# facebookresearch/param

Hardware: AMD Instinct MI355X
Metric: EmbeddingBag lookups/s + achieved HBM GB/s; all-to-all bus-BW at 1/2/4/8 GPU (higher is better)
Workload: dtype f32

## Files before the change

### param_amd/csrc/capi.hip

```cpp
#include <atomic>
#include <cstdio>
#include <cstdlib>
#include <string>

#include "common.h"

namespace {

thread_local std::string g_last_error;

constexpr int kDefaultUnroll = 2;
std::atomic<int> g_unroll{0};
std::atomic<int> g_bags_per_block{0};
std::atomic<int> g_xcd_affine{-1};
std::atomic<int> g_nt_loads{-1};
std::atomic<int> g_stage_out{-1};
std::atomic<int> g_flat_target{-1};
std::atomic<int> g_flat_grid{-1};
constexpr int kDefaultRowPolicy = 3;

int fail(int code, const std::string& msg) {
    g_last_error = msg;
    return code;
}

int hip_fail(hipError_t rc, const char* what) {
    return fail(PM_ERR_HIP, std::string(what) + ": " + hipGetErrorString(rc));
}

struct FwdEnv {
    int stage;
    int flat;
    int flat_maxl;
    int flat_target;
    int flat_bags;
    int tile_major;
    int flat_compact;
};
const FwdEnv& fwd_env() {
    static const FwdEnv e = [] {
        auto num = [](const char* name, int dflt) { const char* v = getenv(name); return v ? atoi(v) : dflt; };
        FwdEnv r;
        const char* st = getenv("PARAM_AMD_FWD_STAGE");
        r.stage = (st && st[0] == '0') ? 0 : 1;
        r.flat = num("PARAM_AMD_FWD_FLAT", 1);
        r.flat_maxl = num("PARAM_AMD_FLAT_MAXL", 0);
        r.flat_target = num("PARAM_AMD_FLAT_TARGET", 256);
        r.flat_bags = num("PARAM_AMD_FLAT_BAGS", 256);
        r.tile_major = num("PARAM_AMD_FWD_TILE_MAJOR", -1);
        r.flat_compact = num("PARAM_AMD_FLAT_COMPACT", 1);
        return r;
    }();
    return e;
}

int flat_target_knob(const FwdEnv& env) { const int k = g_flat_target.load(); return k > 0 ? k : env.flat_target; }

bool dtype_is_weight(int d) { return d == PM_F32 || d == PM_BF16 || d == PM_F16; }

int make_params(const pm_embbag_batch* op, int elem_dtype, pm::KParams& p, bool forward = false) {
    if (!op) return fail(PM_ERR_INVALID, "op is NULL");
    if (op->num_tables < 1) return fail(PM_ERR_INVALID, "num_tables must be >= 1");
    if (!dtype_is_weight(elem_dtype)) return fail(PM_ERR_INVALID, "weight/dst dtype must be PM_F32, PM_BF16 or PM_F16");
    if (op->index_dtype != PM_I64 && op->index_dtype != PM_I32)
        return fail(PM_ERR_INVALID, "index_dtype must be PM_I64 or PM_I32");
    if (op->batch < 0 || op->num_indices < 0) return fail(PM_ERR_INVALID, "negative batch / num_indices");
    if (op->bag_begin < 0 || op->bag_count < 0 || op->bag_begin + op->bag_count > op->batch)
        return fail(PM_ERR_INVALID, "bag_begin/bag_count outside [0, batch]");
    if (!op->tables || !op->rows || !op->dims || !op->out_offsets)
        return fail(PM_ERR_INVALID, "tables/rows/dims/out_offsets must be device pointers");
    if (op->bag_count > 0 && !op->offsets) return fail(PM_ERR_INVALID, "offsets is NULL");
    if (op->num_indices > 0 && !op->indices) return fail(PM_ERR_INVALID, "indices is NULL");
    const int vec = (elem_dtype == PM_F32) ? 4 : 8;
    if (op->max_dim < 1 || op->max_dim % vec != 0)
        return fail(PM_ERR_UNSUPPORTED, "every dims[t] (and max_dim) must be a multiple of " +
                                            std::to_string(vec) + " for this element type");
    if (op->out_stride % 4 != 0) return fail(PM_ERR_UNSUPPORTED, "out_stride must be a multiple of 4 elements");
    if (op->min_dim < 0 || op->min_dim > op->max_dim || (op->min_dim > 0 && op->min_dim % vec != 0))
        return fail(PM_ERR_INVALID, "min_dim must be 0 (not given) or a multiple of the vector width in [1, max_dim]");
    if (op->fixed_pooling < 0 ||
        (op->fixed_pooling > 0 && op->fixed_pooling * op->batch * static_cast<int64_t>(op->num_tables) != op->num_indices))
        return fail(PM_ERR_INVALID, "fixed_pooling must be 0 or num_indices / (num_tables * batch)");

    const int G = pm::group_lanes(op->max_dim, vec);
    const int NG = pm::kBlock / G;
    int bpb = g_bags_per_block.load();
    if (bpb <= 0) {
        bpb = 4 * NG;
        {
            const int64_t tb = static_cast<int64_t>(op->num_tables) * op->batch;
            if (tb > 0 && op->num_indices < 12 * tb) bpb = NG;
        }
        const int64_t want_blocks = 256 * 8;
        while (bpb > NG && static_cast<int64_t>(op->num_tables) * ((op->bag_count + bpb - 1) / bpb) < want_blocks) bpb /= 2;
    }
    if (bpb < NG) bpb = NG;
    if (bpb > 1024) bpb = 1024;

    const int64_t tiles = (op->bag_count + bpb - 1) / bpb;
    if (tiles * op->num_tables > 0x7fffffffLL) return fail(PM_ERR_UNSUPPORTED, "grid too large");

    const int64_t total_bags = static_cast<int64_t>(op->num_tables) * op->batch;
    const int64_t avg_l = total_bags > 0 ? (op->num_indices + total_bags - 1) / total_bags : 0;
    int64_t cap = 2 * bpb * avg_l;
    cap = (cap + 255) / 256 * 256;
    if (cap < (op->per_sample_weights ? 2048 : 4096)) cap = op->per_sample_weights ? 2048 : 4096;
    if (cap > 4096) cap = 4096;

    p.tables = op->tables;
    p.rows = op->rows;
    p.dims = op->dims;
    p.out_offsets = op->out_offsets;
    p.indices = op->indices;
    p.offsets = op->offsets;
    p.psw = op->per_sample_weights;
    p.io = nullptr;
    p.out_stride = op->out_stride;
    p.B = op->batch;
    p.N = op->num_indices;
    p.bag_begin = op->bag_begin;
    p.bag_count = op->bag_count;
    p.T = op->num_tables;
    p.tiles_per_table = static_cast<int32_t>(tiles);
    p.bags_per_block = bpb;
    p.idx_cap = static_cast<int32_t>(cap);
    p.idx64 = op->index_dtype == PM_I64 ? 1 : 0;
    const int xa = g_xcd_affine.load();
    {
        const int64_t tb = static_cast<int64_t>(op->num_tables) * op->batch;
        const bool even_req = tb > 0 && op->num_indices % tb == 0;
        p.xcd_affine = xa == 0 ? 0 : (op->num_tables % pm::kXcds == 0 ? 1 : ((op->num_tables > 1 && even_req) ? 3 : 0));
        if (xa != 0 && op->table_group > 1 && op->num_tables > 1 && even_req) p.xcd_affine = 3;
    }
    const int nt = g_nt_loads.load();
    p.nt_loads = nt > 0 ? nt : 0;
    p.ordered = (total_bags > 0 && op->num_indices % total_bags != 0 && bpb > NG) ? 1 : 0;
    p.alpha = 1.0f;
    if (op->grad_block_shift < 0 || op->grad_block_shift > 31 || op->grad_block_extra < 0 || op->table_group < 0)
        return fail(PM_ERR_INVALID, "grad_block_shift must be in [0, 31], grad_block_extra and table_group >= 0");
    if (op->grad_block_shift == 0 && op->grad_block_extra != 0)
        return fail(PM_ERR_INVALID, "grad_block_extra needs grad_block_shift >= 1 (a block of one bag is the un-blocked layout)");
    if (op->grad_block_shift > 0 && (op->batch & ((static_cast<int64_t>(1) << op->grad_block_shift) - 1)) != 0)
        return fail(PM_ERR_INVALID, "batch must be a multiple of 2^grad_block_shift bags");
    p.gblk_shift = op->grad_block_shift > 0 ? op->grad_block_shift : 31;
    p.gblk_extra = op->grad_block_shift > 0 ? op->grad_block_extra : 0;
    p.out_bits = 0;
    p.stage_out = 0;
    p.stage_bags = 0;
    p.flat_bags = 0;
    p.flat_target = 0;
    p.flat_compact = 0;
    if (forward) {
        const FwdEnv& env = fwd_env();
        int want = g_stage_out.load();
        if (want < 0) want = env.stage;
        const bool even = total_bags > 0 && op->num_indices % total_bags == 0;
        if (want && even && !p.ordered && g_bags_per_block.load() <= 0) {
            while (bpb > NG && static_cast<int64_t>(bpb) * op->max_dim * 4 > 16384) bpb /= 2;
            if (static_cast<int64_t>(bpb) * op->max_dim * 4 <= 16384) {
                const int64_t tiles2 = (op->bag_count + bpb - 1) / bpb;
                if (tiles2 * op->num_tables <= 0x7fffffffLL) {
                    p.bags_per_block = bpb;
                    p.tiles_per_table = static_cast<int32_t>(tiles2);
                    p.stage_out = op->max_dim;
                    int64_t need = (2 * static_cast<int64_t>(bpb) * avg_l + 255) / 256 * 256;
                    if (need < 512) need = 512;
                    if (need < p.idx_cap) p.idx_cap = static_cast<int32_t>(need);
                }
            }
        } else if (want && even && !p.ordered && static_cast<int64_t>(bpb) * op->max_dim * 4 <= 16384) {
            p.stage_out = op->max_dim;
            int64_t need = (2 * static_cast<int64_t>(bpb) * avg_l + 255) / 256 * 256;
            if (need < 512) need = 512;
            if (need < p.idx_cap) p.idx_cap = static_cast<int32_t>(need);
        } else if (want && !even && !p.ordered && g_bags_per_block.load() <= 0 &&
                   static_cast<int64_t>(bpb) * op->max_dim * 4 <= 4096) {
            p.stage_out = op->max_dim;
        }
        p.stage_bags = p.bags_per_block;
        const int flat_env = env.flat;
        const bool flat_on = flat_env != 0;
        const int flat_maxl = env.flat_maxl;
        if (flat_on && even && avg_l <= (flat_maxl > 0 ? flat_maxl : flat_env == 2 ? 4 : 2) && !p.ordered && g_bags_per_block.load() <= 0 &&
            p.stage_out > 0) {
            const int64_t tiles_ng = (op->bag_count + NG - 1) / NG;
            if (tiles_ng * op->num_tables <= 0x7fffffffLL) {
                const int tgt2 = flat_target_knob(env);
                p.flat_bags = env.flat_bags < 32 ? 32 : (env.flat_bags > 1024 ? 1024 : env.flat_bags / NG * NG);
                p.flat_target = tgt2;
                p.tiles_per_table = static_cast<int32_t>(tiles_ng);
                p.stage_bags = NG;
                p.bags_per_block = p.flat_bags;
                if (p.idx_cap < 1024) p.idx_cap = 1024;
            }
        }
        if (flat_on && !even && !p.ordered && g_bags_per_block.load() <= 0 && bpb == NG && p.stage_out > 0) {
            const int cap_env = env.flat_bags;
            const int tgt_env = flat_target_knob(env);
            p.flat_bags = cap_env < NG ? NG : (cap_env > 1024 ? 1024 : cap_env / NG * NG);
            p.flat_target = tgt_env < 1 ? 1 : tgt_env;
            p.bags_per_block = p.flat_bags;
        }
        if (flat_on && op->min_dim > 0 && op->min_dim < op->max_dim && !p.ordered && g_bags_per_block.load() <= 0) {
            int need = (op->min_dim + vec - 1) / vec, g_min = 4;
            while (g_min < need) g_min <<= 1;
            if (g_min < G) {
                const int ng_max = pm::kBlock / g_min;
                const int64_t tiles_ng = (op->bag_count + NG - 1) / NG;
                if (tiles_ng * op->num_tables <= 0x7fffffffLL) {
                    if (p.flat_bags < ng_max) p.flat_bags = ng_max;
                    if (p.flat_bags < 256) p.flat_bags = 256;
                    if (p.flat_bags < 32) p.flat_bags = 32;
                    if (p.flat_target <= 0) p.flat_target = flat_target_knob(env) < 1 ? 1 : flat_target_knob(env);
                    p.tiles_per_table = static_cast<int32_t>(tiles_ng);
                    p.bags_per_block = p.flat_bags;
                    p.stage_out = op->max_dim;
                    p.stage_bags = NG;
                    int64_t cap2 = 2 * static_cast<int64_t>(ng_max) * avg_l;
                    if (cap2 < 2 * static_cast<int64_t>(p.flat_target)) cap2 = 2 * static_cast<int64_t>(p.flat_target);
                    cap2 = (cap2 + 255) / 256 * 256;
                    p.idx_cap = static_cast<int32_t>(cap2 < 1024 ? 1024 : (cap2 > 4096 ? 4096 : cap2));
                    if (p.xcd_affine == 3) p.xcd_affine = 0;
                }
            }
        }
        {
            int fg = g_flat_grid.load();
            if (fg < 0) fg = env.flat_compact;
            if (p.flat_bags > 0 && op->num_tables <= 1024 && fg > 0) {
                const int64_t n_slice = op->batch > 0 ? (op->num_indices * op->bag_count + op->batch - 1) / op->batch : 0;
                const int64_t by_lookups = (n_slice + p.flat_target - 1) / p.flat_target;
                const int64_t by_bags = static_cast<int64_t>(op->num_tables) * ((op->bag_count + p.flat_bags - 1) / p.flat_bags);
                int64_t est = (by_lookups > by_bags ? by_lookups : by_bags) * 5 / 4 + op->num_tables;
                if (est < 1024) est = 1024;
                if (est > (1 << 20)) est = 1 << 20;
                p.flat_compact = fg > 1 ? fg : static_cast<int32_t>(est);
            }
        }
        const int tm_env = env.tile_major;
        const bool uneven = total_bags > 0 && op->num_indices % total_bags != 0;
        if (p.xcd_affine != 1 && op->num_tables > 1 && tm_env > 0 && uneven) p.xcd_affine = 2;
    }
    return PM_OK;
}

int small_request_unroll(const pm_embbag_batch* op, const pm::KParams& p) {
    if (p.flat_bags > 0 || p.ordered) return kDefaultUnroll;
    const int64_t wgs = static_cast<int64_t>(p.T) * p.tiles_per_table;
    const int64_t bags = static_cast<int64_t>(op->num_tables) * op->batch;
    const int64_t avg_l = bags > 0 ? op->num_indices / bags : 0;
    if (wgs > 384) return kDefaultUnroll;
    return avg_l >= 8 ? 8 : (avg_l >= 4 ? 4 : kDefaultUnroll);
}

}

extern "C" {

int pm_abi_version(void) { return PM_ABI_VERSION; }

const char* pm_build_info(void) {
    return "libparam_amd gfx950 (CDNA4, wave64) hip " __VERSION__;
}

const char* pm_last_error(void) { return g_last_error.c_str(); }

int pm_set_tuning(int32_t unroll, int32_t bags_per_block, int32_t xcd_affine, int32_t nt_loads) {
    if (unroll != 0 && unroll != 1 && unroll != 2 && unroll != 3 && unroll != 4 && unroll != 6 && unroll != 8)
        return fail(PM_ERR_INVALID, "unroll must be 0, 1, 2, 3, 4, 6 or 8");
    if (bags_per_block < 0) return fail(PM_ERR_INVALID, "bags_per_block must be >= 0");
    g_unroll.store(unroll);
    g_bags_per_block.store(bags_per_block);
    g_xcd_affine.store(xcd_affine);
    g_nt_loads.store(nt_loads);
    return PM_OK;
}

int pm_set_forward_tuning(int32_t stage_out, int32_t flat_grid, int32_t flat_target) {
    if (stage_out < -1 || stage_out > 1) return fail(PM_ERR_INVALID, "stage_out must be -1, 0 or 1");
    if (flat_grid < -1 || flat_grid > (1 << 20)) return fail(PM_ERR_INVALID, "flat_grid must be -1 (default), 0, 1 or a workgroup count up to 2^20");
    if (flat_target < -1 || flat_target == 0 || flat_target > 4096) return fail(PM_ERR_INVALID, "flat_target must be -1 (default) or 1 .. 4096");
    g_stage_out.store(stage_out);
    g_flat_grid.store(flat_grid);
    g_flat_target.store(flat_target);
    return PM_OK;
}

int pm_set_backward_tuning(int32_t sort_impl, int32_t order, int32_t xcd_affine, int32_t max_phases) {
    if (sort_impl < -1 || sort_impl > 2 || order < -1 || order > 1 || xcd_affine < -1 || xcd_affine > 1)
        return fail(PM_ERR_INVALID, "sort_impl must be -1 .. 2, order / xcd_affine -1, 0 or 1");
#ifndef PM_ALTERNATES
    if (sort_impl > 0)
        return fail(PM_ERR_UNSUPPORTED, "sort_impl 1 (rocPRIM) and 2 (round 2's LSD sort) exist in the alternates build only "
                                        "(libparam_amd_alt.so: make -C param_amd/csrc alt)");
#endif
    if (max_phases != -1 && max_phases != 1 && max_phases != 2) return fail(PM_ERR_INVALID, "max_phases must be -1, 1 or 2");
    pm::set_backward_tuning(sort_impl, order, xcd_affine, max_phases);
    return PM_OK;
}

int pm_set_sort_tuning(int32_t mode) {
    if (mode < -1 || mode > 3) return fail(PM_ERR_INVALID, "mode must be -1, 0, 1, 2 or 3");
    pm::set_sort_tuning(mode);
    return PM_OK;
}

int pm_set_hybrid_tuning(int32_t enable, int64_t lookback_spin_cap) {
    if (enable < -1 || enable > 2) return fail(PM_ERR_INVALID, "enable must be -1 .. 2");
    if (lookback_spin_cap < 0 || lookback_spin_cap > 0xffffffffLL) return fail(PM_ERR_INVALID, "lookback_spin_cap must be in [0, 2^32)");
    pm::set_hybrid_tuning(enable, static_cast<uint32_t>(lookback_spin_cap));
    return PM_OK;
}

int pm_set_hybrid_rest(int32_t mode) {
    if (mode < -1 || mode > 1) return fail(PM_ERR_INVALID, "mode must be -1 (default), 0 or 1");
    pm::set_hybrid_rest(mode);
    return PM_OK;
}

int pm_set_hybrid_min_tiles(int32_t tiles) {
    if (tiles < -1) return fail(PM_ERR_INVALID, "tiles must be -1 (default) or >= 0");
    pm::set_hybrid_min_tiles(tiles);
    return PM_OK;
}

int pm_embbag_sort_status(const pm_embbag_batch* op, int64_t max_rows, const void* workspace, pm_sort_status* out, pm_stream_t stream) {
    pm::KParams p;
    int rc = make_params(op, op ? op->weight_dtype : -1, p);
    if (rc != PM_OK) return rc;
    if (max_rows < 1 || max_rows > (1LL << 31)) return fail(PM_ERR_INVALID, "max_rows must be in [1, 2^31]");
    if (!workspace || !out) return fail(PM_ERR_INVALID, "NULL argument");
    uint32_t v[6] = {0, 0, 0, 0, 0, 0};
    const hipError_t h = pm::sort_status(p, max_rows, op->max_dim, workspace, static_cast<hipStream_t>(stream), v);
    if (h == hipErrorInvalidValue) return fail(PM_ERR_INVALID, "no sort has been recorded for this workspace");
    if (h != hipSuccess) return hip_fail(h, "pm_embbag_sort_status");
    out->lookback_fallbacks = v[0];
    out->pairs_sorted = v[1];
    out->hybrid_tables = v[2];
    out->hybrid_launched = v[3];
    out->lds_pairs = v[4];
    out->lds_tables = v[5];
    return PM_OK;
}

#ifdef PM_ALTERNATES
int64_t pm_radix_sort_scratch_bytes(int64_t n_max) {
    if (n_max < 0 || n_max > 0xffffffffLL) return fail(PM_ERR_INVALID, "n_max must be in [0, 2^32)");
    return static_cast<int64_t>(pm::rs_scratch_bytes(static_cast<size_t>(n_max)));
}

int pm_radix_sort_pairs(void* keys_a, void* keys_b, uint32_t* vals_a, uint32_t* vals_b, int64_t n_max,
                        const uint32_t* d_count, int32_t key_bytes, int32_t begin_bit, int32_t end_bit, int64_t segment_len,
                        void* scratch, int64_t scratch_bytes, int32_t* result_in_b, pm_stream_t stream) {
    if (n_max < 0 || n_max > 0xffffffffLL) return fail(PM_ERR_INVALID, "n_max must be in [0, 2^32)");
    if (key_bytes != 4 && key_bytes != 8) return fail(PM_ERR_INVALID, "key_bytes must be 4 or 8");
    if (begin_bit < 0 || end_bit < begin_bit || end_bit > key_bytes * 8) return fail(PM_ERR_INVALID, "bad bit range");
    if (!result_in_b) return fail(PM_ERR_INVALID, "result_in_b is NULL");
    if (segment_len < 0 || (segment_len > 0 && (segment_len % 4096 != 0 || n_max % segment_len != 0 || d_count)))
        return fail(PM_ERR_INVALID, "segment_len must be 0 or a multiple of 4096 dividing n_max (and d_count NULL)");
    *result_in_b = pm::rs_num_passes(begin_bit, end_bit) % 2;
    if (n_max == 0) return PM_OK;
    if (!keys_a || !keys_b || !vals_a || !vals_b) return fail(PM_ERR_INVALID, "key / value buffers are NULL");
    if (!scratch || scratch_bytes < static_cast<int64_t>(pm::rs_scratch_bytes(static_cast<size_t>(n_max))))
        return fail(PM_ERR_INVALID, "scratch too small: need " + std::to_string(pm::rs_scratch_bytes(static_cast<size_t>(n_max))) + " bytes");
    hipError_t h = key_bytes == 4
        ? pm::rs_sort_pairs<uint32_t>(static_cast<uint32_t*>(keys_a), static_cast<uint32_t*>(keys_b), vals_a, vals_b,
                                      static_cast<size_t>(n_max), d_count, begin_bit, end_bit, scratch, static_cast<hipStream_t>(stream),
                                      static_cast<size_t>(segment_len))
        : pm::rs_sort_pairs<uint64_t>(static_cast<uint64_t*>(keys_a), static_cast<uint64_t*>(keys_b), vals_a, vals_b,
                                      static_cast<size_t>(n_max), d_count, begin_bit, end_bit, scratch, static_cast<hipStream_t>(stream),
                                      static_cast<size_t>(segment_len));
    if (h != hipSuccess) return hip_fail(h, "pm_radix_sort_pairs");
    return PM_OK;
}
#endif

static int rowquant_args_ok(int64_t n_rows, int32_t dim, int32_t bitwidth) {
    if (n_rows < 0) return fail(PM_ERR_INVALID, "n_rows is negative");
    if (bitwidth != 16 && bitwidth != 8 && bitwidth != 4 && bitwidth != 2) return fail(PM_ERR_INVALID, "bitwidth must be 16, 8, 4 or 2");
    if (dim < 8 || dim % 8 != 0 || dim > 512) return fail(PM_ERR_UNSUPPORTED, "dim must be a multiple of 8 in [8, 512]");
    return PM_OK;
}

static uintptr_t rowquant_align(int32_t bitwidth) { return bitwidth == 16 ? 16 : static_cast<uintptr_t>(bitwidth); }

int64_t pm_rows_quantized_bytes(int64_t n_rows, int32_t dim, int32_t bitwidth) {
    const int rc = rowquant_args_ok(n_rows, dim, bitwidth);
    if (rc != PM_OK) return rc;
    return n_rows * pm::rows_quantized_row_bytes(dim, bitwidth);
}

int pm_rows_quantize(const float* src, int64_t n_rows, int32_t dim, int32_t bitwidth, void* dst, pm_stream_t stream) {
    const int rc = rowquant_args_ok(n_rows, dim, bitwidth);
    if (rc != PM_OK) return rc;
// ... 462 lines not shown
```

### param_amd/csrc/common.h

```cpp
#pragma once

#include <hip/hip_runtime.h>
#include <stdint.h>

#include <string>

#include "param_amd.h"

namespace pm {

constexpr int kBlock = 256;
constexpr int kWave = 64;
constexpr int kXcds = 8;

typedef uint32_t u32x4 __attribute__((ext_vector_type(4)));
typedef float f32x4 __attribute__((ext_vector_type(4)));

#define PM_GLOBAL __attribute__((address_space(1)))
template <typename T>
__device__ __forceinline__ const PM_GLOBAL T* as_global(const void* p) { return (const PM_GLOBAL T*)(p); }
template <typename T>
__device__ __forceinline__ PM_GLOBAL T* as_global(void* p) { return (PM_GLOBAL T*)(p); }

struct KParams {
    const void* const* tables;
    const int64_t* rows;
    const int32_t* dims;
    const int64_t* out_offsets;
    const void* indices;
    const void* offsets;
    const float* psw;
    float* io;
    int64_t out_stride;
    int64_t B;
    int64_t N;
    int64_t bag_begin;
    int64_t bag_count;
    int32_t T;
    int32_t tiles_per_table;
    int32_t bags_per_block;
    int32_t idx_cap;
    int32_t idx64;
    int32_t xcd_affine;
    int32_t nt_loads;
    int32_t ordered;
    int32_t stage_out;
    int32_t stage_bags;
    int32_t out_bits;
    int32_t flat_bags;
    int32_t flat_target;
    int32_t flat_compact;
    int32_t gblk_shift;
    int64_t gblk_extra;
    float alpha;
};

__device__ __forceinline__ int64_t grad_bag_offset(int64_t bag, int64_t out_stride, int shift, int64_t extra) {
    int64_t o = bag * out_stride;
    if (__builtin_expect(extra != 0, 0)) o += (bag >> shift) * extra;
    return o;
}

__device__ __forceinline__ int64_t load_index(const void* p, int64_t i, int idx64) {
    return idx64 ? as_global<int64_t>(p)[i] : static_cast<int64_t>(as_global<int32_t>(p)[i]);
}

__device__ __forceinline__ int64_t bag_start_or_end(const KParams& p, int64_t g) {
    const int64_t TB = static_cast<int64_t>(p.T) * p.B;
    return (g < TB) ? load_index(p.offsets, g, p.idx64) : p.N;
}

__device__ __forceinline__ int xcd_contiguous_tile(int bid, int total) {
    const int q = total / kXcds, r = total % kXcds, x = bid % kXcds;
    return x * q + (x < r ? x : r) + bid / kXcds;
}

__device__ __forceinline__ void block_to_tile(const KParams& p, int& t, int& tile, int bid = blockIdx.x) {
    if (p.xcd_affine == 3) {
        const int g = xcd_contiguous_tile(bid, p.T * p.tiles_per_table);
        t = g / p.tiles_per_table;
        tile = g % p.tiles_per_table;
    } else if (p.xcd_affine == 2) {
        t = bid % p.T;
        tile = bid / p.T;
    } else if (p.xcd_affine) {
        const int xcd = bid % kXcds;
        const int slot = bid / kXcds;
        t = xcd + kXcds * (slot / p.tiles_per_table);
        tile = slot % p.tiles_per_table;
    } else {
        t = bid / p.tiles_per_table;
        tile = bid % p.tiles_per_table;
    }
}

template <bool WEIGHTED>
__device__ __forceinline__ bool stage_tile_at(const KParams& p, int t, int64_t bag0, int nb, char* smem,
                                              int64_t*& s_off, int32_t*& s_idx, float*& s_w);

template <bool WEIGHTED>
__device__ __forceinline__ bool stage_tile(const KParams& p, int t, int tile, char* smem, int& nb,
                                           int64_t*& s_off, int32_t*& s_idx, float*& s_w) {
    const int64_t bag0 = p.bag_begin + static_cast<int64_t>(tile) * p.bags_per_block;
    const int64_t left = p.bag_begin + p.bag_count - bag0;
    nb = left < p.bags_per_block ? static_cast<int>(left) : p.bags_per_block;
    return stage_tile_at<WEIGHTED>(p, t, bag0, nb, smem, s_off, s_idx, s_w);
}

template <bool WEIGHTED>
__device__ __forceinline__ bool stage_tile_at(const KParams& p, int t, int64_t bag0, int nb, char* smem,
                                              int64_t*& s_off, int32_t*& s_idx, float*& s_w) {
    const int64_t g0 = static_cast<int64_t>(t) * p.B + bag0;

    s_off = reinterpret_cast<int64_t*>(smem);
    s_idx = reinterpret_cast<int32_t*>(smem + (static_cast<size_t>(p.bags_per_block + 2) / 2 * 2) * sizeof(int64_t));
    s_w = reinterpret_cast<float*>(s_idx + p.idx_cap);

    for (int i = threadIdx.x; i <= nb; i += kBlock) s_off[i] = bag_start_or_end(p, g0 + i);
    __syncthreads();
    const int64_t base = s_off[0];
    const int64_t cnt = s_off[nb] - base;
    const bool staged = cnt <= p.idx_cap;
    if (staged) {
        for (int i = threadIdx.x; i < static_cast<int>(cnt); i += kBlock) {
            s_idx[i] = static_cast<int32_t>(load_index(p.indices, base + i, p.idx64));
            if (WEIGHTED) s_w[i] = as_global<float>(p.psw)[base + i];
        }
        __syncthreads();
    }
    return staged;
}

__host__ __device__ inline size_t tile_lds_bytes(int bags_per_block, int idx_cap, bool weighted) {
    return (static_cast<size_t>(bags_per_block + 2) / 2 * 2) * sizeof(int64_t) +
           static_cast<size_t>(idx_cap) * 4 * (weighted ? 2 : 1);
}

hipError_t launch_embbag_fwd(const KParams& p, int weight_dtype, int max_dim, int unroll,
                             hipStream_t stream);
hipError_t launch_embbag_fwd_split(const KParams& p, int weight_dtype, int max_dim, hipStream_t stream);
hipError_t launch_embbag_psw_grad(const KParams& p, int weight_dtype, int max_dim, int min_dim, float* out, hipStream_t stream);
#ifdef PM_ALTERNATES
hipError_t launch_embbag_bwd(const KParams& p, int dst_dtype, int max_dim, hipStream_t stream);
#endif
hipError_t launch_embbag_check(const KParams& p, int32_t* d_err, int vec, int max_dim, int64_t fixed_pooling,
                               int uniform_dims, hipStream_t stream);
hipError_t launch_fill_random(void* dst, int64_t count, int dtype, int dist, float lo, float hi,
                              uint64_t seed, hipStream_t stream);

hipError_t sorted_workspace_bytes(const KParams& p, int64_t max_rows, int max_dim, size_t& bytes);
hipError_t sort_indices(const KParams& p, int64_t max_rows, int max_dim, int64_t fixed_pooling, int phases, void* workspace,
                        hipStream_t stream, bool defer_ok = false);
int bwd_sorted_plan_check(const KParams& p, int64_t max_rows, const void* workspace, bool adagrad);
int sorted_pairs_info(const KParams& p, int64_t max_rows, int max_dim, const void* workspace, const void** keys, const uint32_t** vals,
                      const uint32_t** d_count, int* key_bytes, int* tshift);
std::string sort_plan_describe(const KParams& p, int64_t max_rows, int64_t fixed_pooling, int phases);
hipError_t bwd_sorted_apply(const KParams& p, int64_t max_rows, int dst_dtype, int max_dim, const void* workspace,
                            float* const* momentum, const pm_rowwise_adagrad* opt, hipStream_t stream,
                            float* const* elem_state = nullptr);

#ifdef PM_ALTERNATES
size_t rs_scratch_bytes(size_t n_max);
int rs_num_passes(int begin_bit, int end_bit);
struct RsSource {
    const void* indices;
    int idx64;
    int tshift;
    uint32_t pooling;
};
template <typename K>
hipError_t rs_sort_pairs(K* keys_a, K* keys_b, uint32_t* vals_a, uint32_t* vals_b, size_t n_max, const uint32_t* d_count,
                         int begin_bit, int end_bit, void* scratch, hipStream_t stream, size_t seg_len = 0,
                         const RsSource* src = nullptr);
#endif

constexpr int kHybMaxTables = 128;
#ifndef PM_BLOOM_K
#define PM_BLOOM_K 4
#endif
constexpr int kBloomK = PM_BLOOM_K;
constexpr int kBloomWords = (1 << 16) / kBloomK;
constexpr int kBloomTableWords = kBloomK * kBloomWords;
constexpr uint32_t kHybMaxCount = 1u << 18;
constexpr int kBloomKMax = 64;
__host__ __device__ inline int hyb_slices(int64_t n_lookups, int T) {
    const int64_t per = T > 0 ? (n_lookups + T - 1) / T : 0;
    int k = PM_BLOOM_K;
    while (k < kBloomKMax && per > static_cast<int64_t>(k) * (kHybMaxCount / PM_BLOOM_K)) k *= 2;
    return k;
}
constexpr uint32_t kHybMinCount = 8192;
constexpr int kUniqueBags = 128;
constexpr int kCompactMaxTiles = 4096;
bool seg_sort_hybrid_available();
struct HybTable {
    uint32_t mode;
    uint32_t pooling;
    uint32_t n_dup;
    uint32_t cand;
};
__host__ __device__ inline uint32_t bloom_word(uint32_t row, int wbits) { return (row * 0x9E3779B1u) >> (32 - wbits); }
__host__ __device__ inline int bloom_wbits(int slices) { int b = 14; while ((1 << (b - 14)) < slices) ++b; return b; }
__host__ __device__ inline uint32_t bloom_mask(uint32_t row) {
    const uint32_t h = row * 0x85EBCA77u;
    return (1u << (h >> 27)) | (1u << ((h >> 22) & 31u)) | (1u << ((h >> 17) & 31u)) | (1u << ((h >> 12) & 31u));
}
struct HybArgs {
    int allow;
    int slices;
};
struct HybTiles {
    int bags_per_tile;
    int tiles_per_table;
};
constexpr int kSegSortMaxTables = 1024;
#ifndef PM_SEG_TILE
#define PM_SEG_TILE 4096
#endif
constexpr int kSegTile = PM_SEG_TILE;
struct SegDesc {
    uint32_t in_start;
    uint32_t count;
    uint32_t out_start;
    uint32_t pooling;
    uint32_t tile_base;
    uint32_t ntiles;
    uint32_t rbits;
    uint32_t pad;
};
struct SegSortRequest {
    const void* indices;
    const void* offsets;
    const int64_t* rows;
    int idx64;
    int T;
    int64_t B, N, bag_begin, bag_count;
    int tshift;
    int rbits_max;
    bool weighted;
    uint32_t* zero4;
    HybArgs hyb;
    uint32_t* queue_a;
    uint32_t* queue_b;
    uint32_t spin_cap;
};
size_t seg_sort_scratch_bytes(size_t n_max, int T, bool hybrid_possible = true);
int seg_sort_radix_bits(int mode, int rbits_max);
bool seg_sort_lookback(int mode, int rbits_max, int64_t n);
int seg_sort_passes(int mode, int rbits_max);
bool seg_sort_result_in_b(int mode, int rbits_max);
const SegDesc* seg_sort_desc(const void* scratch, size_t n_max, int T);
const uint32_t* seg_sort_count(const void* scratch, size_t n_max, int T);
template <typename K>
hipError_t seg_sort_part_a(const SegSortRequest& rq, void* scratch, hipStream_t stream);
template <typename K>
hipError_t seg_sort_part_b(const SegSortRequest& rq, int mode, K* keys_a, K* keys_b, uint32_t* vals_a, uint32_t* vals_b, uint32_t* bag_of,
                           void* scratch, hipStream_t stream, bool hybrid_done = false);
template <typename K>
hipError_t seg_sort_pairs(const SegSortRequest& rq, int mode, K* keys_a, K* keys_b, uint32_t* vals_a, uint32_t* vals_b, uint32_t* bag_of,
                          void* scratch, hipStream_t stream);
const uint32_t* seg_sort_timeouts(const void* scratch, size_t n_max, int T);
const HybTable* seg_sort_hyb_tab(const void* scratch, size_t n_max, int T);
const uint32_t* seg_sort_bloom(const void* scratch, size_t n_max, int T);
uint32_t* seg_sort_tile_cnt(const void* scratch, size_t n_max, int T);
size_t seg_sort_tile_cnt_stride(size_t n_max);
uint32_t* seg_sort_rest_stat(void* scratch, size_t n_max, int T);
constexpr int kRestThreads = 1024;
constexpr int kRestItems = 8;
constexpr int kRestCap = kRestThreads * kRestItems;
const uint32_t* seg_sort_rest_stage(const void* scratch, size_t n_max, int T);
const uint32_t* seg_sort_rest_n(const void* scratch, size_t n_max, int T);
template <typename K>
hipError_t seg_sort_stage_leftovers(const SegSortRequest& rq, const K* keys_b, const uint32_t* vals_b, K* keys_a, uint32_t* vals_a,
                                    HybTiles tiles, int rest_enable, void* scratch, hipStream_t stream);

int64_t rows_quantized_row_bytes(int dim, int bits);
hipError_t launch_rows_quantize(const float* src, int64_t n_rows, int dim, int bits, void* dst, hipStream_t stream);
hipError_t launch_rows_dequantize(const void* src, int64_t n_rows, int dim, int bits, float* dst, hipStream_t stream);
void set_backward_tuning(int sort_impl, int order, int xcd, int max_phases);
void set_sort_tuning(int mode);
void set_hybrid_tuning(int enable, uint32_t spin_cap);
void set_hybrid_min_tiles(int tiles);
void set_hybrid_rest(int mode);
hipError_t sort_status(const KParams& p, int64_t max_rows, int max_dim, const void* workspace, hipStream_t stream, uint32_t out[6]);
struct SparsePairs {
    void* keys;
    int key_bytes;
    int tshift;
    const SegDesc* desc;
// ... 42 lines not shown
```

### param_amd/csrc/embbag_fwd.hip

```cpp
#include <type_traits>

#include "common.h"
#include "fwd_elem.h"
#include "rowquant.inc"

namespace pm {
namespace {

using namespace fwd;

__device__ __forceinline__ float shfl_min(float v, int width) {
    for (int m = width / 2; m >= 1; m >>= 1) v = fminf(v, __shfl_xor(v, m, width));
    return v;
}
__device__ __forceinline__ float shfl_max(float v, int width) {
    for (int m = width / 2; m >= 1; m >>= 1) v = fmaxf(v, __shfl_xor(v, m, width));
    return v;
}

template <int BITS>
__device__ __forceinline__ void fused_rows_burst(const float* s_out, int nb, int D, uint8_t* qout, int64_t row0, int64_t rows_per_bag) {
    int gq = 4;
    while (gq * 8 < D) gq *= 2;
    const int lane = threadIdx.x % gq;
    const int c0 = lane * 4, c1 = (gq + lane) * 4;
    const bool has0 = c0 < D, has1 = c1 < D;
    const int64_t rb = rq::row_bytes(D, BITS);
    for (int r0 = 0; r0 < nb; r0 += kBlock / gq) {
        const int bg = r0 + threadIdx.x / gq;
        const bool live = bg < nb;
        const float* src = s_out + static_cast<size_t>(live ? bg : 0) * D;
        const f32x4 a = has0 ? *reinterpret_cast<const f32x4*>(src + c0) : f32x4{0, 0, 0, 0};
        const f32x4 b = has1 ? *reinterpret_cast<const f32x4*>(src + c1) : f32x4{0, 0, 0, 0};
        float mn, mx;
        rq::row_min_max(a, b, has0, has1, mn, mx);
        mn = shfl_min(mn, gq);
        mx = shfl_max(mx, gq);
        if (!live) continue;
        const float x[8] = {a.x, a.y, a.z, a.w, b.x, b.y, b.z, b.w};
        rq::quantize_row_share<BITS>(x, mn, mx, lane == 0, has0, has1, c0, c1, D, qout + (row0 + bg * rows_per_bag) * rb);
    }
}

__device__ __forceinline__ void quantized_burst(const KParams& p, const float* s_out, int nb, int D, int64_t bag0, int64_t out_off) {
    uint8_t* qout = reinterpret_cast<uint8_t*>(p.io);
    const int64_t rows_per_bag = p.out_stride / D;
    const int64_t row0 = bag0 * rows_per_bag + out_off / D;
    switch (p.out_bits) {
        case 16: {
            typedef uint32_t u32x2 __attribute__((ext_vector_type(2)));
            const int q = D / 4;
            for (int i = threadIdx.x; i < nb * q; i += kBlock) {
                const int bg = i / q, c4 = i % q;
                const f32x4 v = *reinterpret_cast<const f32x4*>(s_out + static_cast<size_t>(bg) * D + c4 * 4);
                u32x2 o;
                o.x = rq::half_bits(v.x) | (static_cast<uint32_t>(rq::half_bits(v.y)) << 16);
                o.y = rq::half_bits(v.z) | (static_cast<uint32_t>(rq::half_bits(v.w)) << 16);
                __builtin_nontemporal_store(o, reinterpret_cast<u32x2*>(qout + (row0 + bg * rows_per_bag) * 2 * D) + c4);
            }
            break;
        }
        case 8: fused_rows_burst<8>(s_out, nb, D, qout, row0, rows_per_bag); break;
        case 4: fused_rows_burst<4>(s_out, nb, D, qout, row0, rows_per_bag); break;
        default: fused_rows_burst<2>(s_out, nb, D, qout, row0, rows_per_bag); break;
    }
}

template <typename WT, int G, int UNROLL, bool WEIGHTED, bool ORDERED, bool STAGE>
__global__ void __launch_bounds__(kBlock) embbag_fwd_kernel(const KParams p) {
    constexpr int VEC = Elem<WT>::kVec;
    constexpr int NG = kBlock / G;
    extern __shared__ __attribute__((aligned(16))) char smem[];
    __shared__ int s_next;

    int t, tile;
    block_to_tile(p, t, tile);
    if (t >= p.T) return;
    const int64_t bag0 = p.bag_begin + static_cast<int64_t>(tile) * p.bags_per_block;
    const int64_t left_bags = p.bag_begin + p.bag_count - bag0;
    const int nb = left_bags < p.bags_per_block ? static_cast<int>(left_bags) : p.bags_per_block;
    if (threadIdx.x == 0) s_next = NG;

    int64_t* s_off;
    int32_t* s_idx;
    float* s_w;
    const bool staged = stage_tile_at<WEIGHTED>(p, t, bag0, nb, smem, s_off, s_idx, s_w);
    const int64_t base = s_off[0];
    __shared__ uint16_t s_ord[ORDERED ? 1024 : 1];
    if (ORDERED) {
        if (nb <= kWave) {
            if (threadIdx.x < kWave) {
                const int i = threadIdx.x;
                int64_t len = i < nb ? s_off[i + 1] - s_off[i] : -1;
                if (len > 0x7fffffffffffLL) len = 0x7fffffffffffLL;
                uint64_t key = (static_cast<uint64_t>(len + 1) << 16) | static_cast<uint64_t>(0xffff - i);
#pragma unroll
                for (int k = 2; k <= kWave; k <<= 1) {
#pragma unroll
                    for (int j = k >> 1; j > 0; j >>= 1) {
                        const uint64_t other = __shfl_xor(key, j, kWave);
                        const bool take_max = ((i & k) == 0) == ((i & j) == 0);
                        key = take_max ? (key > other ? key : other) : (key < other ? key : other);
                    }
                }
                if (i < nb) s_ord[i] = static_cast<uint16_t>(0xffff - (key & 0xffff));
            }
        } else {
            for (int i = threadIdx.x; i < nb; i += kBlock) {
                const int64_t li = s_off[i + 1] - s_off[i];
                int rank = 0;
                for (int j = 0; j < nb; ++j) {
                    const int64_t lj = s_off[j + 1] - s_off[j];
                    rank += (lj > li) || (lj == li && j < i);
                }
                s_ord[rank] = static_cast<uint16_t>(i);
            }
        }
        __syncthreads();
    }
    const int gid = threadIdx.x / G;
    const int lig = threadIdx.x % G;
    const int D = p.dims[t];
    constexpr int ES = 16 / VEC;
    const int64_t row_bytes = static_cast<int64_t>(D) * ES;
    const char* W = reinterpret_cast<const char*>(p.tables[t]);
    float* out_t = p.io + p.out_offsets[t];
    const bool nt = p.nt_loads != 0;
    float* s_out = reinterpret_cast<float*>(smem + tile_lds_bytes(p.bags_per_block, p.idx_cap, WEIGHTED));
    const bool stage = STAGE && nb <= p.stage_bags;

    for (int slot = gid; slot < nb;) {
        const int bg = ORDERED ? s_ord[slot] : slot;
        const int64_t s = s_off[bg];
        const int64_t e = s_off[bg + 1];
        float* orow = out_t + (bag0 + bg) * p.out_stride;

        auto pool = [&](auto staged_c) {
            constexpr bool ST = decltype(staged_c)::value;
            for (int c = lig * VEC; c < D; c += G * VEC) {
                const char* Wc = W + static_cast<int64_t>(c) * ES;
                float acc[VEC];
#pragma unroll
                for (int k = 0; k < VEC; ++k) acc[k] = 0.0f;

                int64_t j = s;
                for (; j + UNROLL <= e; j += UNROLL) {
                    u32x4 raw[UNROLL];
                    float w[UNROLL];
                    int64_t r[UNROLL];
#pragma unroll
                    for (int u = 0; u < UNROLL; ++u) {
                        const int64_t jj = j + u;
                        r[u] = ST ? static_cast<int64_t>(s_idx[jj - base]) : load_index(p.indices, jj, p.idx64);
                        if (WEIGHTED) w[u] = ST ? s_w[jj - base] : as_global<float>(p.psw)[jj];
                    }
#pragma unroll
                    for (int u = 0; u < UNROLL; ++u) raw[u] = load16(Wc + row_offset<ST>(r[u], row_bytes), nt);
#pragma unroll
                    for (int u = 0; u < UNROLL; ++u) {
                        float f[VEC];
                        Elem<WT>::widen(raw[u], f);
#pragma unroll
                        for (int k = 0; k < VEC; ++k) acc[k] = WEIGHTED ? fmaf(w[u], f[k], acc[k]) : acc[k] + f[k];
                    }
                }
                if (j < e) {
                    u32x4 raw[UNROLL];
                    float w[UNROLL];
                    int64_t r[UNROLL];
#pragma unroll
                    for (int u = 0; u < UNROLL - 1; ++u) {
                        const int64_t jj = j + u < e ? j + u : e - 1;
                        r[u] = ST ? static_cast<int64_t>(s_idx[jj - base]) : load_index(p.indices, jj, p.idx64);
                        if (WEIGHTED) w[u] = ST ? s_w[jj - base] : as_global<float>(p.psw)[jj];
                    }
#pragma unroll
                    for (int u = 0; u < UNROLL - 1; ++u) raw[u] = load16(Wc + row_offset<ST>(r[u], row_bytes), nt);
#pragma unroll
                    for (int u = 0; u < UNROLL - 1; ++u) {
                        if (j + u < e) {
                            float f[VEC];
                            Elem<WT>::widen(raw[u], f);
#pragma unroll
                            for (int k = 0; k < VEC; ++k) acc[k] = WEIGHTED ? fmaf(w[u], f[k], acc[k]) : acc[k] + f[k];
                        }
                    }
                }

                if (STAGE && stage) {
                    f32x4* o4 = reinterpret_cast<f32x4*>(s_out + static_cast<size_t>(bg) * D + c);
#pragma unroll
                    for (int k = 0; k < VEC; k += 4) o4[k / 4] = f32x4{acc[k], acc[k + 1], acc[k + 2], acc[k + 3]};
                } else {
                    f32x4* o4 = reinterpret_cast<f32x4*>(orow + c);
#pragma unroll
                    for (int k = 0; k < VEC; k += 4) {
                        f32x4 v = {acc[k], acc[k + 1], acc[k + 2], acc[k + 3]};
                        __builtin_nontemporal_store(v, o4 + k / 4);
                    }
                }
            }
        };
        if (staged) pool(std::true_type{}); else pool(std::false_type{});
        int nxt = 0;
        if (lig == 0) nxt = atomicAdd(&s_next, 1);
        slot = __shfl(nxt, 0, G);
    }
    if (STAGE && stage) {
        __syncthreads();
        if (p.out_bits == 0) {
            const int q = D / 4;
            auto piece = [&](int bg, int c4) {
                const f32x4 v = *reinterpret_cast<const f32x4*>(s_out + static_cast<size_t>(bg) * D + c4 * 4);
                __builtin_nontemporal_store(v, reinterpret_cast<f32x4*>(out_t + (bag0 + bg) * p.out_stride + c4 * 4));
            };
            if ((q & (q - 1)) == 0) {
                const int lg = 31 - __builtin_clz(static_cast<unsigned>(q));
                for (int i = threadIdx.x; i < nb * q; i += kBlock) piece(i >> lg, i & (q - 1));
            } else {
                for (int i = threadIdx.x; i < nb * q; i += kBlock) piece(i / q, i % q);
            }
        } else {
            quantized_burst(p, s_out, nb, D, bag0, p.out_offsets[t]);
        }
    }
}


__host__ __device__ inline size_t flat_tables_offset(const KParams& p, bool weighted) {
    return (tile_lds_bytes(p.bags_per_block, p.idx_cap, weighted) + static_cast<size_t>(p.stage_bags) * p.stage_out * sizeof(float) + 15) / 16 * 16;
}

template <typename WT, int G, int UNROLL, bool WEIGHTED>
// ... 36 lines not shown
        const int64_t row_bytes = static_cast<int64_t>(D) * ES;
        const char* W = reinterpret_cast<const char*>(p.tables[t]);
        float* out_t = p.io + p.out_offsets[t];
        const bool nt = p.nt_loads != 0;
        float* s_out = reinterpret_cast<float*>(smem + tile_lds_bytes(p.bags_per_block, p.idx_cap, WEIGHTED));
        const bool stage = p.stage_out > 0 && static_cast<int64_t>(nb) * D <= static_cast<int64_t>(p.stage_bags) * p.stage_out;
        const int per = (nb + NG - 1) / NG;
        const int b_lo = gid * per;
        const int b_hi = b_lo + per < nb ? b_lo + per : nb;

        auto walk = [&](auto staged_c) {
            constexpr bool ST = decltype(staged_c)::value;
            for (int c = lig * VEC; c < D; c += g * VEC) {
                const char* Wc = W + static_cast<int64_t>(c) * ES;
                float acc[VEC];
#pragma unroll
                for (int k = 0; k < VEC; ++k) acc[k] = 0.0f;
                auto emit = [&](int bg) {
                    if (stage) {
                        f32x4* o4 = reinterpret_cast<f32x4*>(s_out + static_cast<size_t>(bg) * D + c);
#pragma unroll
                        for (int k = 0; k < VEC; k += 4) o4[k / 4] = f32x4{acc[k], acc[k + 1], acc[k + 2], acc[k + 3]};
                    } else {
                        f32x4* o4 = reinterpret_cast<f32x4*>(out_t + (bag0 + bg) * p.out_stride + c);
#pragma unroll
                        for (int k = 0; k < VEC; k += 4) {
                            f32x4 v = {acc[k], acc[k + 1], acc[k + 2], acc[k + 3]};
                            __builtin_nontemporal_store(v, o4 + k / 4);
                        }
                    }
#pragma unroll
                    for (int k = 0; k < VEC; ++k) acc[k] = 0.0f;
                };
                int cur = b_lo;
                int64_t cur_end = s_off[cur + 1];
                const int64_t e = s_off[b_hi];
                for (int64_t j = s_off[b_lo]; j < e; j += UNROLL) {
                    u32x4 raw[UNROLL];
                    float w[UNROLL];
                    int64_t r[UNROLL];
#pragma unroll
                    for (int u = 0; u < UNROLL; ++u) {
                        const int64_t jj = j + u < e ? j + u : e - 1;
                        r[u] = ST ? static_cast<int64_t>(s_idx[jj - base]) : load_index(p.indices, jj, p.idx64);
                        if (WEIGHTED) w[u] = ST ? s_w[jj - base] : as_global<float>(p.psw)[jj];
                    }
#pragma unroll
                    for (int u = 0; u < UNROLL; ++u) raw[u] = load16(Wc + row_offset<ST>(r[u], row_bytes), nt);
#pragma unroll
                    for (int u = 0; u < UNROLL; ++u) {
                        if (j + u < e) {
                            while (j + u >= cur_end) {
                                emit(cur);
                                ++cur;
                                cur_end = s_off[cur + 1];
                            }
                            float f[VEC];
                            Elem<WT>::widen(raw[u], f);
#pragma unroll
                            for (int k = 0; k < VEC; ++k) acc[k] = WEIGHTED ? fmaf(w[u], f[k], acc[k]) : acc[k] + f[k];
                        }
                    }
                }
                for (; cur < b_hi; ++cur) emit(cur);
            }
        };
        if (b_lo < b_hi) {
            if (staged) walk(std::true_type{}); else walk(std::false_type{});
        }
        if (stage) {
            __syncthreads();
            const int q = D / 4;
            for (int i = threadIdx.x; i < nb * q; i += kBlock) {
                const int bg = i / q, c4 = i % q;
                const f32x4 v = *reinterpret_cast<const f32x4*>(s_out + static_cast<size_t>(bg) * D + c4 * 4);
                __builtin_nontemporal_store(v, reinterpret_cast<f32x4*>(out_t + (bag0 + bg) * p.out_stride + c4 * 4));
            }
        }
    };

    const bool compact = p.flat_compact > 0;
    if (compact) {
        for (int t = threadIdx.x; t < p.T; t += kBlock) {
            int D, g, bags;
            geometry(t, D, g, bags);
            s_bags[t] = static_cast<uint16_t>(bags);
            s_pref[t + 1] = static_cast<int>((p.bag_count + bags - 1) / bags);
        }
        __syncthreads();
        if (threadIdx.x < kWave) {
            int running = 0;
            for (int b0 = 0; b0 < p.T; b0 += kWave) {
                const int i = b0 + static_cast<int>(threadIdx.x);
                int v = i < p.T ? s_pref[i + 1] : 0;
#pragma unroll
                for (int d = 1; d < kWave; d <<= 1) {
                    const int o = __shfl_up(v, d, kWave);
                    if (static_cast<int>(threadIdx.x) >= d) v += o;
                }
                if (i < p.T) s_pref[i + 1] = running + v;
                running += __shfl(v, kWave - 1, kWave);
            }
            if (threadIdx.x == 0) s_pref[0] = 0;
        }
        __syncthreads();
    }
    const int total = compact ? s_pref[p.T] : static_cast<int>(blockIdx.x) + 1;
    const int step = compact ? static_cast<int>(gridDim.x) : 1;
    for (int v = blockIdx.x; v < total; v += step) {
        int t, tile, D, g, bags;
        if (compact) {
            int lo = 0, hi = p.T;
            while (hi - lo > 1) {
                const int mid = (lo + hi) >> 1;
                if (s_pref[mid] <= v) lo = mid; else hi = mid;
            }
            t = lo;
            tile = v - s_pref[t];
            D = p.dims[t];
            g = kBlock / p.flat_bags;
            if (g < 1) g = 1;
            while (g < G && g * VEC < D) g <<= 1;
            bags = s_bags[t];
        } else {
            block_to_tile(p, t, tile);
            if (t >= p.T) return;
            geometry(t, D, g, bags);
        }
        do_tile(t, tile, D, g, bags);
        if (compact) __syncthreads();
    }
}

template <typename WT, int G, int UNROLL>
hipError_t launch_w(const KParams& p, hipStream_t stream) {
    const bool weighted = p.psw != nullptr;
    const int grid = p.T * p.tiles_per_table;
    size_t lds = tile_lds_bytes(p.bags_per_block, p.idx_cap, weighted);
    if (p.flat_bags > 0) {
        lds += static_cast<size_t>(p.stage_bags) * p.stage_out * sizeof(float);
        if (p.flat_compact > 0) {
            lds = flat_tables_offset(p, weighted) + static_cast<size_t>(p.T + 1) * 4 + static_cast<size_t>(p.T) * 2;
            const int g2 = p.flat_compact < grid ? p.flat_compact : grid;
            if (weighted) hipLaunchKernelGGL((embbag_fwd_flat_kernel<WT, G, UNROLL, true>), dim3(g2), dim3(kBlock), lds, stream, p);
            else hipLaunchKernelGGL((embbag_fwd_flat_kernel<WT, G, UNROLL, false>), dim3(g2), dim3(kBlock), lds, stream, p);
            return hipGetLastError();
        }
        if (weighted) hipLaunchKernelGGL((embbag_fwd_flat_kernel<WT, G, UNROLL, true>), dim3(grid), dim3(kBlock), lds, stream, p);
        else hipLaunchKernelGGL((embbag_fwd_flat_kernel<WT, G, UNROLL, false>), dim3(grid), dim3(kBlock), lds, stream, p);
        return hipGetLastError();
    }
#define PM_FWD(W_, O_, S_) hipLaunchKernelGGL((embbag_fwd_kernel<WT, G, UNROLL, W_, O_, S_>), dim3(grid), dim3(kBlock), lds, stream, p)
    if (p.stage_out && !p.ordered) {
        lds += static_cast<size_t>(p.bags_per_block) * p.stage_out * sizeof(float);
        if (weighted) PM_FWD(true, false, true); else PM_FWD(false, false, true);
    } else if (weighted) { if (p.ordered) PM_FWD(true, true, false); else PM_FWD(true, false, false); }
    else { if (p.ordered) PM_FWD(false, true, false); else PM_FWD(false, false, false); }
#undef PM_FWD
    return hipGetLastError();
}

template <typename WT, int G>
hipError_t launch_u(const KParams& p, int unroll, hipStream_t stream) {
    switch (unroll) {
        case 1: return launch_w<WT, G, 1>(p, stream);
        case 2: return launch_w<WT, G, 2>(p, stream);
        case 3: return launch_w<WT, G, 3>(p, stream);
        case 4: return launch_w<WT, G, 4>(p, stream);
        case 6: return launch_w<WT, G, 6>(p, stream);
        default: return launch_w<WT, G, 8>(p, stream);
    }
}

template <typename WT>
hipError_t launch_g(const KParams& p, int max_dim, int unroll, hipStream_t stream) {
    switch (group_lanes(max_dim, Elem<WT>::kVec)) {
        case 8: return launch_u<WT, 8>(p, unroll, stream);
        case 16: return launch_u<WT, 16>(p, unroll, stream);
        case 32: return launch_u<WT, 32>(p, unroll, stream);
        default: return launch_u<WT, 64>(p, unroll, stream);
    }
}

}

hipError_t launch_embbag_fwd(const KParams& p, int weight_dtype, int max_dim, int unroll,
                             hipStream_t stream) {
    switch (weight_dtype) {
        case PM_F32: return launch_g<float>(p, max_dim, unroll, stream);
        case PM_BF16: return launch_g<bf16_t>(p, max_dim, unroll, stream);
        default: return launch_g<f16_t>(p, max_dim, unroll, stream);
    }
}

}
```

Baseline: 21.95 billion.

## Tighten staged index LDS capacity and add optional half-size tail tiles

Adds a tighter sizing rule for the staged index buffer. It uses roughly bpb*avg_l plus slack instead of twice that, when the resulting LDS footprint fits an eighth of 160KB, so more blocks can share a CU. It also adds an opt-in tail-half scheme, off by default, which splits the last table per XCD into half-size bag tiles to balance the work in the final wave. The tight cap is on by default and shrinks headroom for index staging, which may matter if bag lengths vary.

```diff
diff --git a/param_amd/csrc/capi.hip b/param_amd/csrc/capi.hip
--- a/param_amd/csrc/capi.hip
+++ b/param_amd/csrc/capi.hip
@@ -10,6 +10,7 @@
 thread_local std::string g_last_error;
 
 constexpr int kDefaultUnroll = 2;
+constexpr int kDefaultFwdTail = 0;
 std::atomic<int> g_unroll{0};
 std::atomic<int> g_bags_per_block{0};
 std::atomic<int> g_xcd_affine{-1};
@@ -36,6 +37,8 @@
     int flat_bags;
     int tile_major;
     int flat_compact;
+    int idx_tight;
+    int tail;
 };
 const FwdEnv& fwd_env() {
     static const FwdEnv e = [] {
@@ -49,9 +52,23 @@
         r.flat_bags = num("PARAM_AMD_FLAT_BAGS", 256);
         r.tile_major = num("PARAM_AMD_FWD_TILE_MAJOR", -1);
         r.flat_compact = num("PARAM_AMD_FLAT_COMPACT", 1);
+        r.idx_tight = num("PARAM_AMD_FWD_IDXCAP", 1);
+        r.tail = num("PARAM_AMD_FWD_TAIL", kDefaultFwdTail);
         return r;
     }();
     return e;
+}
+
+int64_t staged_idx_cap(int bpb, int64_t avg_l, int max_dim, bool weighted, bool tight) {
+    int64_t need = (2 * static_cast<int64_t>(bpb) * avg_l + 255) / 256 * 256;
+    if (need < 512) need = 512;
+    if (tight) {
+        int64_t snug = (static_cast<int64_t>(bpb) * avg_l + 128 + 127) / 128 * 128;
+        if (snug < 512) snug = 512;
+        const size_t lds = pm::tile_lds_bytes(bpb, static_cast<int>(snug), weighted) + static_cast<size_t>(bpb) * max_dim * sizeof(float);
+        if (snug < need && lds + pm::kFwdStaticLds <= pm::kFwdLdsPerEighth) need = snug;
+    }
+    return need;
 }
 
 int flat_target_knob(const FwdEnv& env) { const int k = g_flat_target.load(); return k > 0 ? k : env.flat_target; }
@@ -147,6 +164,7 @@
     p.out_bits = 0;
     p.stage_out = 0;
     p.stage_bags = 0;
+    p.tail_half = 0;
     p.flat_bags = 0;
     p.flat_target = 0;
     p.flat_compact = 0;
@@ -163,15 +181,13 @@
                     p.bags_per_block = bpb;
                     p.tiles_per_table = static_cast<int32_t>(tiles2);
                     p.stage_out = op->max_dim;
-                    int64_t need = (2 * static_cast<int64_t>(bpb) * avg_l + 255) / 256 * 256;
-                    if (need < 512) need = 512;
+                    const int64_t need = staged_idx_cap(bpb, avg_l, op->max_dim, op->per_sample_weights != nullptr, env.idx_tight != 0);
                     if (need < p.idx_cap) p.idx_cap = static_cast<int32_t>(need);
                 }
             }
         } else if (want && even && !p.ordered && static_cast<int64_t>(bpb) * op->max_dim * 4 <= 16384) {
             p.stage_out = op->max_dim;
-            int64_t need = (2 * static_cast<int64_t>(bpb) * avg_l + 255) / 256 * 256;
-            if (need < 512) need = 512;
+            const int64_t need = staged_idx_cap(bpb, avg_l, op->max_dim, op->per_sample_weights != nullptr, env.idx_tight != 0);
             if (need < p.idx_cap) p.idx_cap = static_cast<int32_t>(need);
         } else if (want && !even && !p.ordered && g_bags_per_block.load() <= 0 &&
                    static_cast<int64_t>(bpb) * op->max_dim * 4 <= 4096) {
@@ -240,6 +256,9 @@
         const int tm_env = env.tile_major;
         const bool uneven = total_bags > 0 && op->num_indices % total_bags != 0;
         if (p.xcd_affine != 1 && op->num_tables > 1 && tm_env > 0 && uneven) p.xcd_affine = 2;
+        if (env.tail > 0 && p.xcd_affine == 1 && p.stage_out > 0 && !p.ordered && p.flat_bags == 0 && p.bags_per_block % 2 == 0 &&
+            p.bags_per_block / 2 >= NG && pm::fwd_tile_grid(p) + pm::kXcds * static_cast<int64_t>(p.tiles_per_table) <= 0x7fffffffLL)
+            p.tail_half = 1;
     }
     return PM_OK;
 }
diff --git a/param_amd/csrc/common.h b/param_amd/csrc/common.h
--- a/param_amd/csrc/common.h
+++ b/param_amd/csrc/common.h
@@ -47,6 +47,7 @@
     int32_t stage_out;
     int32_t stage_bags;
     int32_t out_bits;
+    int32_t tail_half;
     int32_t flat_bags;
     int32_t flat_target;
     int32_t flat_compact;
@@ -94,6 +95,27 @@
     }
 }
 
+__device__ __forceinline__ int block_to_tile_bags(const KParams& p, int& t, int& tile, int bid = blockIdx.x) {
+    if (p.tail_half && p.xcd_affine == 1) {
+        const int xcd = bid % kXcds;
+        const int slot = bid / kXcds;
+        const int full = (p.T / kXcds - 1) * p.tiles_per_table;
+        if (slot >= full) {
+            t = p.T - kXcds + xcd;
+            tile = slot - full;
+            return p.bags_per_block / 2;
+        }
+        t = xcd + kXcds * (slot / p.tiles_per_table);
+        tile = slot % p.tiles_per_table;
+        return p.bags_per_block;
+    }
+    block_to_tile(p, t, tile, bid);
+    return p.bags_per_block;
+}
+__host__ __device__ inline int64_t fwd_tile_grid(const KParams& p) {
+    return static_cast<int64_t>(p.T) * p.tiles_per_table + (p.tail_half ? static_cast<int64_t>(kXcds) * p.tiles_per_table : 0);
+}
+
 template <bool WEIGHTED>
 __device__ __forceinline__ bool stage_tile_at(const KParams& p, int t, int64_t bag0, int nb, char* smem,
                                               int64_t*& s_off, int32_t*& s_idx, float*& s_w);
@@ -135,6 +157,8 @@
     return (static_cast<size_t>(bags_per_block + 2) / 2 * 2) * sizeof(int64_t) +
            static_cast<size_t>(idx_cap) * 4 * (weighted ? 2 : 1);
 }
+constexpr size_t kFwdLdsPerEighth = 160 * 1024 / 8;
+constexpr size_t kFwdStaticLds = 16;
 
 hipError_t launch_embbag_fwd(const KParams& p, int weight_dtype, int max_dim, int unroll,
                              hipStream_t stream);
diff --git a/param_amd/csrc/embbag_fwd.hip b/param_amd/csrc/embbag_fwd.hip
--- a/param_amd/csrc/embbag_fwd.hip
+++ b/param_amd/csrc/embbag_fwd.hip
@@ -74,11 +74,13 @@
     __shared__ int s_next;
 
     int t, tile;
-    block_to_tile(p, t, tile);
+    int tile_bags = p.bags_per_block;
+    if (STAGE) tile_bags = block_to_tile_bags(p, t, tile); else block_to_tile(p, t, tile);
     if (t >= p.T) return;
-    const int64_t bag0 = p.bag_begin + static_cast<int64_t>(tile) * p.bags_per_block;
+    const int64_t bag0 = p.bag_begin + static_cast<int64_t>(tile) * tile_bags;
     const int64_t left_bags = p.bag_begin + p.bag_count - bag0;
-    const int nb = left_bags < p.bags_per_block ? static_cast<int>(left_bags) : p.bags_per_block;
+    if (STAGE && left_bags <= 0) return;
+    const int nb = left_bags < tile_bags ? static_cast<int>(left_bags) : tile_bags;
     if (threadIdx.x == 0) s_next = NG;
 
     int64_t* s_off;
@@ -421,6 +423,7 @@
     }
 #define PM_FWD(W_, O_, S_) hipLaunchKernelGGL((embbag_fwd_kernel<WT, G, UNROLL, W_, O_, S_>), dim3(grid), dim3(kBlock), lds, stream, p)
     if (p.stage_out && !p.ordered) {
+        const int grid = static_cast<int>(fwd_tile_grid(p));
         lds += static_cast<size_t>(p.bags_per_block) * p.stage_out * sizeof(float);
         if (weighted) PM_FWD(true, false, true); else PM_FWD(false, false, true);
     } else if (weighted) { if (p.ordered) PM_FWD(true, true, false); else PM_FWD(true, false, false); }
```

After: 21.11 billion. -3.8%, worse.
